# LIA-DiTella/DiffUDF

Hardware: AMD Instinct MI355X
Metric: train points/sec (SIREN fwd+∇x+Eikonal loss+bwd), 256×8 net, 100k pts (higher is better)
Workload: dtype f32

## Files before the change

diffudf_amd/csrc/dudf_sweep_bf16.hip:

```cpp
#include "dudf_sweep16.h"


namespace {

template <int H, int SW, int FL, int SP = 0, int P24 = 0>
__device__ __forceinline__ void sweep_tile_b(const SweepArgs& a, const int g_first, const int nact, char* lds, unsigned& gc,
                                             const bool stamp_on = false) {
    using G = GeoB<H, SP>;
    constexpr int NPC = G::NPC;
    static_assert(SP == 0 || SW <= SWEEP_FWD_J, "fp16x3: plain columns, Hessian quads, jets");
    static_assert(P24 == 0 || ((P24 == 6 || P24 == 7) && SP != 0 && H == 256 && !is_jet(SW)), "24-bit stash arrays (mask 6: R, E, C; 7: S, Q, A, Z as well): the fp16x3 training kernels of 256-wide layers");
    constexpr int BS = base_of(SW);
    constexpr bool HS = is_hess(SW);
    const int tid = threadIdx.x, lane = tid & 63;
    const int wave = __builtin_amdgcn_readfirstlane(tid >> 6);
    const int li = lane & 15, q = lane >> 4;
    const bool isv = !HS || (is_jet(SW) ? li == 0 : (lane & 3) == 0);
    const int nhid = a.L - 1;
    constexpr bool kFwdDir = (BS == SWEEP_FWD || BS == SWEEP_ADJ_FWD);

    f32x4 acc[G::NT], prev[G::NT];
    const int64_t p = (int64_t)(g_first + wave) * 16 + li;
    auto image = [&](int j) -> const char* {
        if constexpr (SP) return kFwdDir ? a.wimg16_f + (size_t)j * G::IMGB : a.wimg16_t + (size_t)(nhid - 1 - j) * G::IMGB;
        return kFwdDir ? a.wimg_f + (size_t)j * G::IMGB : a.wimg_t + (size_t)(nhid - 1 - j) * G::IMGB;
    };
    float unscale = 1.f;
    auto unscale_of = [&](int j) -> float { return a.wsc[kFwdDir ? j : nhid - 1 - j]; };
    constexpr bool kColScale = SP != 0 && (BS != SWEEP_FWD || HS);
    constexpr bool kTrackE = SP != 0 && BS == SWEEP_ADJ_FWD;
    float sb = 1.f, inv_sb = 1.f;
    auto set_scale = [&](float amax_true, float extra, float zb) {
        float bound;
        if constexpr (!HS) { (void)zb; bound = a.w0 * amax_true + extra; }
        else if constexpr (is_jet(SW)) {
            const int l0 = lane & 48;
            const unsigned jw = kJetLane[lane & 15];
            const float w2 = 0.5f * (float)((jw >> 24) & 3), w3 = 0.5f * (float)((jw >> 26) & 3);
            const float F[3] = {a.w0 * __shfl(amax_true, l0 + 1), a.w0 * __shfl(amax_true, l0 + 2), a.w0 * __shfl(amax_true, l0 + 3)};
            auto sel = [&](unsigned k) -> float { k &= 3; return k == 0 ? F[0] : (k == 1 ? F[1] : F[2]); };
            const float S0 = a.w0 * __shfl(amax_true, l0 + (int)(jw & 15)), S1 = a.w0 * __shfl(amax_true, l0 + (int)((jw >> 4) & 15)),
                        S2 = a.w0 * __shfl(amax_true, l0 + (int)((jw >> 8) & 15));
            const float fab = sel(jw >> 18) * sel(jw >> 20);
            const float p2 = S0 * sel(jw >> 12) + S1 * sel(jw >> 14) + S2 * sel(jw >> 16) + w2 * fab;
            const float p3 = w3 * fab * sel(jw >> 22);
            bound = ((jw >> 28) & 1) ? 1.f : a.w0 * amax_true + p3 + p2;
        }
        else if constexpr (BS == SWEEP_FWD) bound = isv ? 1.f : a.w0 * amax_true;
        else if constexpr (BS == SWEEP_REV) {
            const float av = quad_bcast0(amax_true);
            bound = a.w0 * (amax_true + (isv ? 0.f : a.w0 * zb * av));
        } else {
            const float sk = quad_sum(isv ? 0.f : zb * amax_true);
            bound = extra + a.w0 * (amax_true + (isv ? a.w0 * sk : 0.f));
        }
        col_scale(bound * DUDF_FX_HEADROOM, sb, inv_sb);
    };
    auto ebound_of = [&](int layer) -> float {
        if constexpr (kColScale && BS == SWEEP_ADJ_REV && (HS || (FL & 1) != 0)) return a.ebound[(int64_t)layer * a.np + p];
        return 0.f;
    };
    auto zbound_of = [&](int layer) -> float {
        if constexpr (kColScale && HS && BS != SWEEP_FWD) return a.zbound[(int64_t)layer * a.nch + p];
        return 0.f;
    };
    auto store_zbound = [&](int layer, float m) {
        if constexpr (kColScale && HS && !is_jet(SW) && BS == SWEEP_FWD) a.zbound[(int64_t)layer * a.nch + p] = isv ? 0.f : m;
    };
    float eb_next = 0.f, zb_next = 0.f;
    constexpr int kRow = amax_row<SW, FL>();
    constexpr bool kFx = (P24 & 1) != 0;
    TailTrackT<kFx> tmax;
    bool poison = false;
    auto store_fx = [&](int layer) {
        if constexpr (kFx) {
            if constexpr (kColScale) tmax.fs = sb * 0x1p-15f;
            if constexpr (kColScale) a.fxs[(int64_t)layer * a.np + p] = poison ? __uint_as_float(0x7fc00000u) : inv_sb * 0x1p15f;
        }
    };
    unsigned* lds_amax = reinterpret_cast<unsigned*>(lds + amax_lds_off<H, SW, SP>(a));
    auto publish = [&](int layer) {
        if constexpr (kRow >= 0) { lds_max_wave(lds_amax + (layer < kMaxAmaxLayers ? layer : kMaxAmaxLayers - 1), tmax.t); tmax.t = 0.f; }
    };
    auto in_layer = [&](int j) -> int { return kFwdDir ? j : a.L - 1 - j; };
    auto bias_ptr = [&](int layer) -> const float* {
        return a.b1s + (size_t)layer * H;
    };
    auto stash_base = [&](int layer, int T) -> int64_t {
        const int64_t v = (int64_t)layer * a.stash_layer + (int64_t)(16 * T) * a.np;
        const unsigned lo = __builtin_amdgcn_readfirstlane((unsigned)v), hi = __builtin_amdgcn_readfirstlane((unsigned)(v >> 32));
        return (int64_t)(((uint64_t)hi << 32) | lo);
    };
    const unsigned vo = (unsigned)(((int64_t)q * a.np + p) * 16);
    const LaneOff vl(vo, (is_hess(SW) && !is_jet(SW)) ? (unsigned)(((int64_t)q * a.np + (p >> 2)) * 16) : vo,
                     P24 ? (unsigned)(((p >> 4) * 64 + lane) * 12) : 0u,
                     !P24 ? 0u : (is_hess(SW) && !is_jet(SW)) ? (unsigned)(((p >> 6) * 64 + 16 * q + ((p >> 2) & 15)) * 12)
                                                              : (unsigned)(((p >> 4) * 64 + lane) * 12));
    auto load_ops = [&](int layer, int kb, TailOps& o) {
        epilogue_loads<SW, FL, P24>(a, stash_base(layer, 2 * kb), vl, o.o1a, o.o2a, o.o3a);
        epilogue_loads<SW, FL, P24>(a, stash_base(layer, 2 * kb + 1), vl, o.o1b, o.o2b, o.o3b);
        if constexpr (BS == SWEEP_FWD && SP != 0) {
            const float* lb = reinterpret_cast<const float*>(lds + 3 * G::CHUNKB) + layer * H + 32 * kb + 4 * q;
            o.ba = *reinterpret_cast<const f32x4*>(lb);
            o.bb = *reinterpret_cast<const f32x4*>(lb + 16);
        } else if constexpr (BS == SWEEP_FWD) {
            o.ba = *reinterpret_cast<const f32x4*>(bias_ptr(layer) + 32 * kb + 4 * q);
            o.bb = *reinterpret_cast<const f32x4*>(bias_ptr(layer) + 32 * kb + 16 + 4 * q);
        }
    };
    auto run_tail = [&](int layer, int kb, const f32x4 z0, const f32x4 z1, const TailOps& o, f32x4& e0, f32x4& e1) {
        const f32x4 zero = {0, 0, 0, 0};
        if constexpr (BS == SWEEP_FWD && SP != 0 && HS) {
            const f32x4 us = {unscale, unscale, unscale, unscale};
            e0 = epilogue<SW, FL, false, P24, false, TailTrackT<kFx>>(a, __builtin_elementwise_fma(z0, us, isv ? o.ba : zero), zero, zero, zero, stash_base(layer, 2 * kb), vl, isv, tmax);
            e1 = epilogue<SW, FL, false, P24, false, TailTrackT<kFx>>(a, __builtin_elementwise_fma(z1, us, isv ? o.bb : zero), zero, zero, zero, stash_base(layer, 2 * kb + 1), vl, isv, tmax);
        } else if constexpr (BS == SWEEP_FWD && SP != 0) {
            e0 = epilogue<SW, FL, false, P24, false, TailTrackT<kFx>>(a, __builtin_elementwise_fma(z0, f32x4{unscale, unscale, unscale, unscale}, o.ba), zero, zero, zero, stash_base(layer, 2 * kb), vl, isv, tmax);
            e1 = epilogue<SW, FL, false, P24, false, TailTrackT<kFx>>(a, __builtin_elementwise_fma(z1, f32x4{unscale, unscale, unscale, unscale}, o.bb), zero, zero, zero, stash_base(layer, 2 * kb + 1), vl, isv, tmax);
        } else if constexpr (BS == SWEEP_FWD) {
            e0 = epilogue<SW, FL, false, P24, false, TailTrackT<kFx>>(a, z0 + (isv ? o.ba : zero), zero, zero, zero, stash_base(layer, 2 * kb), vl, isv, tmax);
            e1 = epilogue<SW, FL, false, P24, false, TailTrackT<kFx>>(a, z1 + (isv ? o.bb : zero), zero, zero, zero, stash_base(layer, 2 * kb + 1), vl, isv, tmax);
        } else if constexpr (kColScale) {
            e0 = epilogue<SW, FL, kTrackE, P24, false, TailTrackT<kFx>>(a, z0 * unscale, o.o1a, o.o2a, o.o3a, stash_base(layer, 2 * kb), vl, isv, tmax);
            e1 = epilogue<SW, FL, kTrackE, P24, false, TailTrackT<kFx>>(a, z1 * unscale, o.o1b, o.o2b, o.o3b, stash_base(layer, 2 * kb + 1), vl, isv, tmax);
        } else {
            e0 = epilogue<SW, FL, false, P24, false, TailTrackT<kFx>>(a, z0, o.o1a, o.o2a, o.o3a, stash_base(layer, 2 * kb), vl, isv, tmax);
            e1 = epilogue<SW, FL, false, P24, false, TailTrackT<kFx>>(a, z1, o.o1b, o.o2b, o.o3b, stash_base(layer, 2 * kb + 1), vl, isv, tmax);
        }
    };
    auto pin_ops = [&](TailOps& o) {
        if constexpr (BS == SWEEP_FWD) asm volatile("" : "+v"(o.ba), "+v"(o.bb));
        else asm volatile("" : "+v"(o.o1a), "+v"(o.o2a), "+v"(o.o1b), "+v"(o.o2b));
        if constexpr (SW == SWEEP_ADJ_FWD_H || SW == SWEEP_ADJ_REV_H) asm volatile("" : "+v"(o.o3a), "+v"(o.o3b));
    };

    const int total = nhid * G::NKB;
    auto chunk_src = [&](int c) -> const char* {
        const int j = c / G::NKB;
        return image(j) + (size_t)(c - j * G::NKB) * G::CHUNKB;
    };
    __syncthreads();
    const unsigned lds0 = (unsigned)(size_t)(__attribute__((address_space(3))) char*)lds;
    const unsigned voff = (unsigned)lane * 16u;
    auto dma2 = [&](const char* src, unsigned dst) {
        if (wave < NWB / 2) {
            const int w = wave & (NWB / 2 - 1);
            dma_issue<H, SP>(src, dst, voff, w); dma_issue<H, SP>(src, dst, voff, w + NWB / 2);
        }
    };
    dma2(chunk_src(0), lds0 + gc * G::CHUNKB);
    dma2(chunk_src(1), lds0 + ((gc + 1) % 3) * G::CHUNKB);
    if (wave >= nact) {
        dma_wait_b<0>();
        __syncthreads();
        for (int c = 0; c < total; ++c) {
            const bool more = c + 2 < total;
            if (more) dma2(chunk_src(c + 2), lds0 + ((gc + 2) % 3) * G::CHUNKB);
            gc = (gc + 1) % 3;
            if (more) dma_wait_b<2 * G::NDMA>();
            else dma_wait_b<0>();
            __syncthreads();
        }
        return;
    }

    {
        float b = 0.f, yb = 1.f;
        if constexpr (BS == SWEEP_FWD) b = (q < 3) ? a.x4[p * 4 + q] : 0.f;
        if constexpr (BS == SWEEP_ADJ_FWD) b = (q < 3) ? a.gbar[p * 4 + q] : 0.f;
        if constexpr (BS == SWEEP_ADJ_REV) yb = a.ybar[p];
        if constexpr (SW == SWEEP_REV_H) yb = isv ? 1.f : 0.f;
        if constexpr (kFx) {
            if constexpr (BS == SWEEP_REV) poison = nonfinite(a.y[p]);
            if constexpr (BS == SWEEP_ADJ_REV) poison = nonfinite(a.ybar[p]);
            if constexpr (BS == SWEEP_ADJ_FWD) {
                int bad = nonfinite(b) ? 1 : 0;
                bad |= __shfl_xor(bad, 16); bad |= __shfl_xor(bad, 32);
                poison = bad != 0;
            }
        }
#pragma unroll
        for (int T = 0; T < G::NT; ++T) {
            if constexpr (kFwdDir) prev[T] = mfma16(a.w1b[(16 * T + li) * 4 + q], b, f32x4{0, 0, 0, 0});
            else prev[T] = *reinterpret_cast<const f32x4*>(a.theta + a.off_wo + 16 * T + 4 * q) * yb;
        }
    }

    constexpr bool kOneSet = HS;
    TailOps ops_cur, ops_n1;
    u32x4 bp[NPC];
    auto split = [&](const f32x4 e0, const f32x4 e1, u32x4 (&o)[NPC]) {
        if constexpr (kColScale) split8h(e0 * sb, e1 * sb, o[0], o[1]);
        else if constexpr (SP) split8h(e0, e1, o[0], o[1]);
        else split8(e0, e1, o[0], o[1], o[2]);
    };
    auto store_ebound = [&](int layer) {
        if constexpr (kTrackE) {
            float m = fmaxf(tmax.e, __shfl_xor(tmax.e, 16));
            m = fmaxf(m, __shfl_xor(m, 32));
            a.ebound[(int64_t)layer * a.np + p] = m;
            tmax.e = 0.f;
        }
    };
    f32x4 fin0 = {0, 0, 0, 0}, fin1 = {0, 0, 0, 0};
    load_ops(in_layer(0), 0, ops_cur);
    if constexpr (!kOneSet) load_ops(in_layer(0), 1, ops_n1);
    if constexpr (kColScale) {
        const float eb0 = ebound_of(in_layer(0)), zb0 = zbound_of(in_layer(0));
        if (nhid > 0) { eb_next = ebound_of(in_layer(1)); zb_next = zbound_of(in_layer(1)); }
        const float cm = col_absmax(prev);
        store_zbound(in_layer(0), cm);
        set_scale(cm, eb0, zb0);
    }
    store_fx(in_layer(0));
    {
        f32x4 e0, e1;
        run_tail(in_layer(0), 0, prev[0], prev[1], ops_cur, e0, e1);
        split(e0, e1, bp);
        if constexpr (kOneSet) load_ops(in_layer(0), 1, ops_cur);
    }
#pragma unroll
    for (int T = 0; T < G::NT; ++T) acc[T] = f32x4{0, 0, 0, 0};
    dma_wait_b<0>();
    __syncthreads();
    constexpr int kYoung = younger_ops<SW, FL>() - ((SP != 0 && BS == SWEEP_FWD) ? 2 : 0);
    constexpr bool kLateOk = !HS || (SW != SWEEP_ADJ_FWD_H && SW != SWEEP_FWD_J);
    #ifdef DUDF_LATE_FORCE
    const bool late = kLateOk && DUDF_LATE_FORCE;
#else
    const bool late = kLateOk && __builtin_amdgcn_readfirstlane((int)(wave >= NWB / 2)) != 0;
#endif
    constexpr int FA = -1, TA = 0, FB = (BS == SWEEP_FWD ? 15 : 7) * (G::NT - 1) / 15, TB = G::NT - 1;
    for (int j = 0; j < nhid; ++j) {
        const int lin = in_layer(j), lnx = in_layer(j + 1);
#pragma unroll
        for (int kb = 0; kb < G::NKB; ++kb) {
            const int c = j * G::NKB + kb;
            const char* bpl = lds + gc * G::CHUNKB + lane * 16;
            auto frag = [&](int T, int pc) -> u32x4 {
#if DUDF_SWEEP_DBG & 32
                u32x4 z; asm volatile("" : "=v"(z)); return z;
#endif
                return *reinterpret_cast<const u32x4*>(bpl + (T * NPC + pc) * G::FRAG);
            };
            DUDF_STAMP(0);
            if constexpr (!kOneSet) ops_cur = ops_n1;
            pin_ops(ops_cur);
            const bool more = c + 2 < total;
            auto load_after_next = [&](TailOps& o) {
                if (kb + 2 < G::NKB) load_ops(lin, kb + 2, o);
                else load_ops(lnx, kb + 2 - G::NKB, o);
            };
            auto feed = [&]() {
                if (more) dma2(chunk_src(c + 2), lds0 + ((gc + 2) % 3) * G::CHUNKB);
                if constexpr (!kOneSet) load_after_next(ops_n1);
            };
            u32x4 nb[NPC];
            constexpr bool kTailTop = SP != 0 && BS == SWEEP_FWD;
            if (kTailTop && !late && kb + 1 < G::NKB) {
                DUDF_STAMP(2);
                f32x4 e0, e1;
                run_tail(lin, kb + 1, prev[2 * kb + 2], prev[2 * kb + 3], ops_cur, e0, e1);
                split(e0, e1, nb);
                if constexpr (kOneSet) load_after_next(ops_cur);
                DUDF_STAMP(3);
                __builtin_amdgcn_sched_barrier(0);
            }
            if ((FA < 0 && !late) || (FB < 0 && late)) feed();
            DUDF_STAMP(1);
            __builtin_amdgcn_sched_barrier(0);
            constexpr int AD = (SP && BS == SWEEP_FWD) ? 4 : 2;
            u32x4 an[AD][NPC];
#pragma unroll
            for (int T = 0; T < AD; ++T)
#pragma unroll
                for (int pc = 0; pc < NPC; ++pc) an[T][pc] = frag(T, pc);
            constexpr int TP = SP ? 2 : 1;
#pragma unroll
            for (int T = 0; T < G::NT; T += TP) {
                u32x4 af[TP][NPC];
#pragma unroll
                for (int u = 0; u < TP; ++u)
#pragma unroll
                    for (int pc = 0; pc < NPC; ++pc) af[u][pc] = an[(T + u) % AD][pc];
                if (T + AD < G::NT) {
#pragma unroll
                    for (int u = 0; u < TP; ++u)
#pragma unroll
                        for (int pc = 0; pc < NPC; ++pc) an[(T + u) % AD][pc] = frag(T + u + AD, pc);
                    __builtin_amdgcn_sched_barrier(0x76);
                }
                f32x4 cc[TP];
#pragma unroll
                for (int u = 0; u < TP; ++u) cc[u] = acc[T + u];
                if constexpr (SP) {
#pragma unroll
                    for (int u = 0; u < TP; ++u) cc[u] = mfma_h(as_h(af[u][1]), as_h(bp[0]), cc[u]);
#pragma unroll
                    for (int u = 0; u < TP; ++u) cc[u] = mfma_h(as_h(af[u][0]), as_h(bp[1]), cc[u]);
#pragma unroll
                    for (int u = 0; u < TP; ++u) cc[u] = mfma_h(as_h(af[u][0]), as_h(bp[0]), cc[u]);
                } else {
#pragma unroll
                    for (int u = 0; u < TP; ++u) cc[u] = mfma_b(as_bf(af[u][1]), as_bf(bp[1]), cc[u]);
#pragma unroll
                    for (int u = 0; u < TP; ++u) cc[u] = mfma_b(as_bf(af[u][2]), as_bf(bp[0]), cc[u]);
#pragma unroll
                    for (int u = 0; u < TP; ++u) cc[u] = mfma_b(as_bf(af[u][0]), as_bf(bp[2]), cc[u]);
#pragma unroll
                    for (int u = 0; u < TP; ++u) cc[u] = mfma_b(as_bf(af[u][1]), as_bf(bp[0]), cc[u]);
#pragma unroll
                    for (int u = 0; u < TP; ++u) cc[u] = mfma_b(as_bf(af[u][0]), as_bf(bp[1]), cc[u]);
#pragma unroll
                    for (int u = 0; u < TP; ++u) cc[u] = mfma_b(as_bf(af[u][0]), as_bf(bp[0]), cc[u]);
                }
#pragma unroll
                for (int u = 0; u < TP; ++u) acc[T + u] = cc[u];
                const int Tl = T + TP - 1;
                if ((FA >= T && FA <= Tl && !late) || (FB >= T && FB <= Tl && late)) {
                    __builtin_amdgcn_sched_barrier(0);
                    DUDF_STAMP(6);
                    feed();
                    DUDF_STAMP(7);
                    __builtin_amdgcn_sched_barrier(0);
                }
                if (kb + 1 < G::NKB && ((TA >= T && TA <= Tl && !late && !kTailTop) || (TB >= T && TB <= Tl && late))) {
                    if (T != 0) __builtin_amdgcn_sched_barrier(0);
                    DUDF_STAMP(2);
                    f32x4 e0, e1;
                    run_tail(lin, kb + 1, prev[2 * kb + 2], prev[2 * kb + 3], ops_cur, e0, e1);
                    split(e0, e1, nb);
                    if constexpr (kOneSet) load_after_next(ops_cur);
                    DUDF_STAMP(3);
                }
            }
            if (kb + 1 == G::NKB) {
                if constexpr (kColScale) {
                    unscale = unscale_of(j) * inv_sb;
                    const float ebl = eb_next, zbl = zb_next;
                    { const int jn = j + 2 <= nhid ? j + 2 : nhid; eb_next = ebound_of(in_layer(jn)); zb_next = zbound_of(in_layer(jn)); }
                    const float cm = col_absmax(acc) * unscale;
                    store_zbound(lnx, cm);
                    set_scale(cm, ebl, zbl);
                } else if constexpr (SP) unscale = unscale_of(j);
                store_fx(lnx);
                publish(lin);
                store_ebound(lin);
                run_tail(lnx, 0, acc[0], acc[1], ops_cur, fin0, fin1);
                split(fin0, fin1, nb);
                if constexpr (kOneSet) load_after_next(ops_cur);
#pragma unroll
                for (int T = 0; T < G::NT; ++T) { prev[T] = acc[T]; acc[T] = f32x4{0, 0, 0, 0}; }
            }
#pragma unroll
            for (int pc = 0; pc < NPC; ++pc) bp[pc] = nb[pc];
            gc = (gc + 1) % 3;
            DUDF_STAMP(4);
#if !(DUDF_SWEEP_DBG & 8)
            if (more) { if (wave < NWB / 2) dma_wait_b<(kTailTop ? 1 : 2) * kYoung + 2 * G::NDMA>(); }
            else dma_wait_b<0>();
#endif
            DUDF_STAMP(5);
#if !(DUDF_SWEEP_DBG & 16)
            __syncthreads();
#endif
        }
    }

    {
        const int lin = in_layer(nhid);
        float part = 0.f;
        f32x4 accg = {0, 0, 0, 0};
#pragma unroll
        for (int kb = 0; kb < G::NKB; ++kb) {
            f32x4 e0 = fin0, e1 = fin1;
            if (kb > 0) {
                if constexpr (!kOneSet) {
                    ops_cur = ops_n1;
                    if (kb + 1 < G::NKB) load_ops(lin, kb + 1, ops_n1);
                }
                run_tail(lin, kb, prev[2 * kb], prev[2 * kb + 1], ops_cur, e0, e1);
                if constexpr (kOneSet) { if (kb + 1 < G::NKB) load_ops(lin, kb + 1, ops_cur); }
            }
            if constexpr (BS == SWEEP_FWD) {
                const f32x4 w0v = *reinterpret_cast<const f32x4*>(a.theta + a.off_wo + 32 * kb + 4 * q);
                const f32x4 w1v = *reinterpret_cast<const f32x4*>(a.theta + a.off_wo + 32 * kb + 16 + 4 * q);
                part += e0[0] * w0v[0] + e0[1] * w0v[1] + e0[2] * w0v[2] + e0[3] * w0v[3];
                part += e1[0] * w1v[0] + e1[1] * w1v[1] + e1[2] * w1v[2] + e1[3] * w1v[3];
            } else if constexpr (BS == SWEEP_REV) {
                const f32x4 w0v = *reinterpret_cast<const f32x4*>(a.w1t16 + li * H + 32 * kb + 4 * q);
                const f32x4 w1v = *reinterpret_cast<const f32x4*>(a.w1t16 + li * H + 32 * kb + 16 + 4 * q);
#pragma unroll
                for (int t = 0; t < 4; ++t) accg = mfma16(w0v[t], e0[t], accg);
#pragma unroll
                for (int t = 0; t < 4; ++t) accg = mfma16(w1v[t], e1[t], accg);
            }
        }
        publish(lin);
        store_ebound(lin);
        if constexpr (BS == SWEEP_FWD) {
            part += __shfl_xor(part, 16);
            part += __shfl_xor(part, 32);
            if (isv) part += a.theta[a.off_bo];
            if (q == 0) a.y[p] = part;
            if constexpr (kFx) {
                if constexpr (kColScale) {
                    if (q == 0 && nonfinite(part))
                        for (int l = 0; l < a.L; ++l) a.fxs[(int64_t)l * a.np + p] = __uint_as_float(0x7fc00000u);
                } else if (q == 0) {
                    const float sc = nonfinite(part) ? __uint_as_float(0x7fc00000u) : 1.f;
                    for (int l = 0; l < a.L; ++l) a.fxs[(int64_t)l * a.np + p] = sc;
                }
            }
        } else if constexpr (BS == SWEEP_REV) {
            if constexpr (kFx) { if (poison) accg = f32x4{__uint_as_float(0x7fc00000u), __uint_as_float(0x7fc00000u), __uint_as_float(0x7fc00000u), 0.f}; }
            if (q == 0) *reinterpret_cast<f32x4*>(a.g + p * 4) = f32x4{accg[0], accg[1], accg[2], 0.f};
        }
    }
}

template <int H, int SW, int FL, int P24 = 0>
__device__ __forceinline__ void sweep_tile_oct(const SweepArgs& a, const int g, char* lds, unsigned& gc, const unsigned oct_off) {
    using G = GeoB<H, 1>;
    static_assert(H == 256 && SW <= SWEEP_ADJ_REV, "fp16x3, plain columns, one k-block per wave");
    constexpr int NPC = 2;
    constexpr int BS = base_of(SW);
    const int tid = threadIdx.x, lane = tid & 63;
    const int wave = __builtin_amdgcn_readfirstlane(tid >> 6);
    const int li = lane & 15, q = lane >> 4;
    const int nhid = a.L - 1;
    constexpr bool kFwdDir = (BS == SWEEP_FWD || BS == SWEEP_ADJ_FWD);
    constexpr bool kColScale = BS != SWEEP_FWD;
    constexpr bool kTrackE = BS == SWEEP_ADJ_FWD;
    constexpr int kRow = amax_row<SW, FL>();
    const int64_t p = (int64_t)g * 16 + li;
    const int T0 = 2 * wave;
    auto image = [&](int j) -> const char* {
        return kFwdDir ? a.wimg16_f + (size_t)j * G::IMGB : a.wimg16_t + (size_t)(nhid - 1 - j) * G::IMGB;
    };
    auto unscale_of = [&](int j) -> float { return a.wsc[kFwdDir ? j : nhid - 1 - j]; };
    auto in_layer = [&](int j) -> int { return kFwdDir ? j : a.L - 1 - j; };
    auto stash_base = [&](int layer, int T) -> int64_t {
        const int64_t v = (int64_t)layer * a.stash_layer + (int64_t)(16 * T) * a.np;
        const unsigned lo = __builtin_amdgcn_readfirstlane((unsigned)v), hi = __builtin_amdgcn_readfirstlane((unsigned)(v >> 32));
        return (int64_t)(((uint64_t)hi << 32) | lo);
    };
    const LaneOff vo((unsigned)(((int64_t)q * a.np + p) * 16), (unsigned)(((int64_t)q * a.np + p) * 16),
                     P24 ? (unsigned)(((p >> 4) * 64 + lane) * 12) : 0u);
    char* ox = lds + oct_off;
    u32x4* Bx = reinterpret_cast<u32x4*>(ox);
    float* cmx = reinterpret_cast<float*>(ox + 8 * NPC * 1024);
    float* emx = cmx + 128;
    f32x4* red = reinterpret_cast<f32x4*>(ox + 8 * NPC * 1024 + 1024);
    unsigned* lds_amax = reinterpret_cast<unsigned*>(lds + 3 * G::CHUNKB);

    (void)gc;
    __syncthreads();

    f32x4 prev[2], acc[2];
    bool poison = false;
    {
        float b = 0.f, yb = 1.f;
        if constexpr (BS == SWEEP_FWD) b = (q < 3) ? a.x4[p * 4 + q] : 0.f;
        if constexpr (BS == SWEEP_ADJ_FWD) b = (q < 3) ? a.gbar[p * 4 + q] : 0.f;
        if constexpr (BS == SWEEP_ADJ_REV) yb = a.ybar[p];
        if constexpr ((P24 & 1) != 0) {
            if constexpr (BS == SWEEP_REV) poison = nonfinite(a.y[p]);
            if constexpr (BS == SWEEP_ADJ_REV) poison = nonfinite(yb);
            if constexpr (BS == SWEEP_ADJ_FWD) {
                int bad = nonfinite(b) ? 1 : 0;
                bad |= __shfl_xor(bad, 16); bad |= __shfl_xor(bad, 32);
                poison = bad != 0;
            }
        }
#pragma unroll
        for (int u = 0; u < 2; ++u) {
            const int T = T0 + u;
            if constexpr (kFwdDir) prev[u] = mfma16(a.w1b[(16 * T + li) * 4 + q], b, f32x4{0, 0, 0, 0});
            else prev[u] = *reinterpret_cast<const f32x4*>(a.theta + a.off_wo + 16 * T + 4 * q) * yb;
        }
    }
    f32x4 o1[2], o2[2], o3[2], bs[2] = {{0, 0, 0, 0}, {0, 0, 0, 0}};
    auto load_ops = [&](int layer) {
#pragma unroll
        for (int u = 0; u < 2; ++u) {
            epilogue_loads<SW, FL, P24>(a, stash_base(layer, T0 + u), vo, o1[u], o2[u], o3[u]);
            if constexpr (BS == SWEEP_FWD)
                bs[u] = *reinterpret_cast<const f32x4*>(reinterpret_cast<const float*>(lds + 3 * G::CHUNKB) + layer * H + 16 * (T0 + u) + 4 * q);
        }
    };
    auto ebound_of = [&](int layer) -> float {
        if constexpr (BS == SWEEP_ADJ_REV && (FL & 1) != 0) return a.ebound[(int64_t)layer * a.np + p];
        return 0.f;
    };
    load_ops(in_layer(0));
    float eb = ebound_of(in_layer(0));
    float unscale = 1.f, sb = 1.f, inv_sb = 1.f;
    constexpr bool kFx = (P24 & 1) != 0;
    TailTrackT<kFx> tk;
    f32x4 e[2];
    for (int j = 0; j <= nhid; ++j) {
        const int lin = in_layer(j);
        if constexpr (kColScale) {
            const float m = col_absmax(prev);
            if (q == 0) cmx[wave * 16 + li] = m;
            __syncthreads();
            float mm = 0.f;
#pragma unroll
            for (int w = 0; w < NWB; ++w) mm = fmaxf(mm, cmx[w * 16 + li]);
            col_scale((a.w0 * (mm * unscale) + eb) * DUDF_FX_HEADROOM, sb, inv_sb);
        }
        if constexpr (kFx) {
            if constexpr (kColScale) tk.fs = sb * 0x1p-15f;
            if (wave == 0 && q == 0) a.fxs[(int64_t)lin * a.np + p] = poison ? __uint_as_float(0x7fc00000u) : (kColScale ? inv_sb * 0x1p15f : 1.f);
        }
#pragma unroll
        for (int u = 0; u < 2; ++u) {
            f32x4 z = prev[u];
            if constexpr (BS == SWEEP_FWD) z = __builtin_elementwise_fma(z, f32x4{unscale, unscale, unscale, unscale}, bs[u]);
            else z *= unscale;
            e[u] = epilogue<SW, FL, kTrackE, P24, false, TailTrackT<kFx>>(a, z, o1[u], o2[u], o3[u], stash_base(lin, T0 + u), vo, true, tk);
        }
        if constexpr (kRow >= 0) { if (lin < kMaxAmaxLayers) lds_max_wave(lds_amax + lin, tk.t); tk.t = 0.f; }
        if constexpr (kTrackE) {
            float m = fmaxf(tk.e, __shfl_xor(tk.e, 16));
            m = fmaxf(m, __shfl_xor(m, 32));
            if (q == 0) emx[wave * 16 + li] = m;
            tk.e = 0.f;
        }
        if (j == nhid) break;
        u32x4 fr[G::NKB][2][NPC];
        {
            const char* img = image(j) + (size_t)lane * 16;
#pragma unroll
            for (int kb = 0; kb < G::NKB; ++kb)
#pragma unroll
                for (int u = 0; u < 2; ++u)
#pragma unroll
                    for (int pc = 0; pc < NPC; ++pc)
                        fr[kb][u][pc] = *reinterpret_cast<const u32x4*>(img + (size_t)kb * G::CHUNKB + ((T0 + u) * NPC + pc) * G::FRAG);
        }
        u32x4 bh, bl;
        if constexpr (kColScale) split8h(e[0] * sb, e[1] * sb, bh, bl);
        else split8h(e[0], e[1], bh, bl);
        Bx[(wave * NPC + 0) * 64 + lane] = bh;
        Bx[(wave * NPC + 1) * 64 + lane] = bl;
        load_ops(in_layer(j + 1));
        eb = ebound_of(in_layer(j + 1));
        __syncthreads();
        if constexpr (kTrackE) {
            if (wave == 0 && q == 0 && a.ebound) {
                float m = 0.f;
#pragma unroll
                for (int w = 0; w < NWB; ++w) m = fmaxf(m, emx[w * 16 + li]);
                a.ebound[(int64_t)lin * a.np + p] = m;
            }
        }
        acc[0] = f32x4{0, 0, 0, 0}; acc[1] = acc[0];
#pragma unroll
        for (int kb = 0; kb < G::NKB; ++kb) {
            const u32x4 b0 = Bx[(kb * NPC + 0) * 64 + lane], b1 = Bx[(kb * NPC + 1) * 64 + lane];
#pragma unroll
            for (int u = 0; u < 2; ++u) {
                f32x4 cc = acc[u];
                cc = mfma_h(as_h(fr[kb][u][1]), as_h(b0), cc);
                cc = mfma_h(as_h(fr[kb][u][0]), as_h(b1), cc);
                cc = mfma_h(as_h(fr[kb][u][0]), as_h(b0), cc);
                acc[u] = cc;
            }
        }
        __syncthreads();
        prev[0] = acc[0]; prev[1] = acc[1];
        unscale = kColScale ? unscale_of(j) * inv_sb : unscale_of(j);
    }
    if constexpr (BS == SWEEP_FWD) {
        float part = 0.f;
#pragma unroll
        for (int u = 0; u < 2; ++u) {
            const f32x4 wv = *reinterpret_cast<const f32x4*>(a.theta + a.off_wo + 16 * (T0 + u) + 4 * q);
            part += e[u][0] * wv[0] + e[u][1] * wv[1] + e[u][2] * wv[2] + e[u][3] * wv[3];
        }
        part += __shfl_xor(part, 16);
        part += __shfl_xor(part, 32);
        if (q == 0) cmx[wave * 16 + li] = part;
        __syncthreads();
        if (wave == 0 && q == 0) {
            float y = a.theta[a.off_bo];
#pragma unroll
            for (int w = 0; w < NWB; ++w) y += cmx[w * 16 + li];
            a.y[p] = y;
            if constexpr (kFx) {
                if (nonfinite(y))
                    for (int l = 0; l < a.L; ++l) a.fxs[(int64_t)l * a.np + p] = __uint_as_float(0x7fc00000u);
            }
        }
    } else if constexpr (BS == SWEEP_REV) {
        f32x4 accg = {0, 0, 0, 0};
#pragma unroll
        for (int u = 0; u < 2; ++u) {
            const f32x4 wv = *reinterpret_cast<const f32x4*>(a.w1t16 + li * H + 16 * (T0 + u) + 4 * q);
#pragma unroll
            for (int t = 0; t < 4; ++t) accg = mfma16(wv[t], e[u][t], accg);
        }
        red[wave * 64 + lane] = accg;
        __syncthreads();
        if (wave == 0 && q == 0) {
            f32x4 sum = {0, 0, 0, 0};
#pragma unroll
            for (int w = 0; w < NWB; ++w) sum += red[w * 64 + lane];
            if constexpr (kFx) { if (poison) sum = f32x4{__uint_as_float(0x7fc00000u), __uint_as_float(0x7fc00000u), __uint_as_float(0x7fc00000u), 0.f}; }
            *reinterpret_cast<f32x4*>(a.g + p * 4) = f32x4{sum[0], sum[1], sum[2], 0.f};
        }
    } else if constexpr (kTrackE) {
        __syncthreads();
        if (wave == 0 && q == 0 && a.ebound) {
            float m = 0.f;
#pragma unroll
            for (int w = 0; w < NWB; ++w) m = fmaxf(m, emx[w * 16 + li]);
            a.ebound[(int64_t)in_layer(nhid) * a.np + p] = m;
        }
    }
}

template <int H, int SW, int FL, int SP = 0, int P24 = 0>
__device__ __forceinline__ void sweep_body_b(const SweepArgs& a, const int bid, const int nblk) {
    extern __shared__ __attribute__((aligned(16))) char lds_b[];
    unsigned gc = 0;
    const bool clk_on = a.clk != nullptr && bid == 0;
    const unsigned long long clk_t0 = clk_on ? __builtin_amdgcn_s_memtime() : 0ull, clk_r0 = clk_on ? __builtin_amdgcn_s_memrealtime() : 0ull;
    constexpr int kRow = amax_row<SW, FL>();
    unsigned* lds_amax = reinterpret_cast<unsigned*>(lds_b + amax_lds_off<H, SW, SP>(a));
    if constexpr (kRow >= 0) { if (threadIdx.x < kMaxAmaxLayers) lds_amax[threadIdx.x] = 0u; }
    if constexpr (SP != 0 && base_of(SW) == SWEEP_FWD) {
        float* lb = reinterpret_cast<float*>(lds_b + 3 * GeoB<H, SP>::CHUNKB);
        for (int i = threadIdx.x; i < a.L * H; i += 64 * NWB) lb[i] = a.b1s[i];
    }
    const int ng = a.ntiles * (TILE / 16), gbase = a.tile0 * (TILE / 16);
    const int g0 = (int)((int64_t)bid * ng / nblk), g1 = (int)((int64_t)(bid + 1) * ng / nblk);
    constexpr bool kOct = SP != 0 && H == 256 && SW <= SWEEP_ADJ_REV;
    for (int g = g0; g < g1; g += NWB) {
        if constexpr (kOct) {
            if (g1 - g == 1) {
                const unsigned oct_off = 3 * GeoB<H, SP>::CHUNKB + (base_of(SW) == SWEEP_FWD ? (unsigned)(a.L * H * sizeof(float)) : (unsigned)(kMaxAmaxLayers * sizeof(unsigned)));
                sweep_tile_oct<H, SW, FL, P24>(a, gbase + g, lds_b, gc, oct_off);
                continue;
            }
        }
        sweep_tile_b<H, SW, FL, SP, P24>(a, gbase + g, (g1 - g < NWB) ? g1 - g : NWB, lds_b, gc, (DUDF_SWEEP_DBG & 128) && bid == 100 && g == g0);
    }
    if constexpr (kRow >= 0) {
        __syncthreads();
        if ((int)threadIdx.x < a.L && (int)threadIdx.x < kMaxAmaxLayers && a.amax) {
            const unsigned v = lds_amax[threadIdx.x];
            if (v) atomicMax(a.amax + kRow * a.L + threadIdx.x, v);
        }
    }
    if (clk_on && threadIdx.x == 0) {
        a.clk[0] = __builtin_amdgcn_s_memtime() - clk_t0;
        a.clk[1] = __builtin_amdgcn_s_memrealtime() - clk_r0;
    }
}
template <int H, int SW, int FL>
__global__ __launch_bounds__(64 * NWB) void sweep_bf16_kernel(SweepArgs a) { sweep_body_b<H, SW, FL>(a, blockIdx.x, gridDim.x); }
template <int H, int SW, int FL>
__global__ __launch_bounds__(64 * NWB) DUDF_NO_PK void sweep_bf16_np_kernel(SweepArgs a) { sweep_body_b<H, SW, FL>(a, blockIdx.x, gridDim.x); }
template <int H, int SW, int FL>
__global__ __launch_bounds__(64 * NWB) void sweep_f16_kernel(SweepArgs a) { sweep_body_b<H, SW, FL, 1>(a, blockIdx.x, gridDim.x); }
template <int H, int SW, int FL>
__global__ __launch_bounds__(64 * NWB) DUDF_NO_PK void sweep_f16_np_kernel(SweepArgs a) { sweep_body_b<H, SW, FL, 1>(a, blockIdx.x, gridDim.x); }
template <int H, int SW, int FL>
__global__ __launch_bounds__(64 * NWB) void sweep_f16r_kernel(SweepArgs a) { sweep_body_b<H, SW, FL, 1, 6>(a, blockIdx.x, gridDim.x); }
template <int H, int SW, int FL>
__global__ __launch_bounds__(64 * NWB) DUDF_NO_PK void sweep_f16r_np_kernel(SweepArgs a) { sweep_body_b<H, SW, FL, 1, 6>(a, blockIdx.x, gridDim.x); }
template <int H, int SW, int FL>
__global__ __launch_bounds__(64 * NWB) void sweep_f16p_kernel(SweepArgs a) { sweep_body_b<H, SW, FL, 1, 7>(a, blockIdx.x, gridDim.x); }
template <int H, int SW, int FL>
__global__ __launch_bounds__(64 * NWB) DUDF_NO_PK void sweep_f16p_np_kernel(SweepArgs a) { sweep_body_b<H, SW, FL, 1, 7>(a, blockIdx.x, gridDim.x); }
template <int H, int SWQ, int FLQ, int SWP, int FLP, int SPQ, int P24 = 0>
__global__ __launch_bounds__(64 * NWB) DUDF_NO_PK void sweep_pair_kernel(SweepArgs aq, SweepArgs ap, int nbq) {
    if ((int)blockIdx.x < nbq) sweep_body_b<H, SWQ, FLQ, SPQ, P24>(aq, blockIdx.x, nbq);
    else sweep_body_b<H, SWP, FLP, 1, P24>(ap, (int)blockIdx.x - nbq, (int)gridDim.x - nbq);
}

template <int H, int FAM, int SW, int FL>
constexpr auto sweep_kernel_of() {
    constexpr bool np = sweep_no_pk<SW>();
    if constexpr (FAM == DUDF_FAM_BF16) { if constexpr (np) return &sweep_bf16_np_kernel<H, SW, FL>; else return &sweep_bf16_kernel<H, SW, FL>; }
    else if constexpr (FAM == DUDF_FAM_F16) { if constexpr (np) return &sweep_f16_np_kernel<H, SW, FL>; else return &sweep_f16_kernel<H, SW, FL>; }
    else if constexpr (FAM == DUDF_FAM_F16R) { if constexpr (np) return &sweep_f16r_np_kernel<H, SW, FL>; else return &sweep_f16r_kernel<H, SW, FL>; }
    else { if constexpr (np) return &sweep_f16p_np_kernel<H, SW, FL>; else return &sweep_f16p_kernel<H, SW, FL>; }
}
static_assert(dudf_chunk_bytes(256, 3) == GeoB<256>::CHUNKB && dudf_chunk_bytes(128, 2) == GeoB<128, 1>::CHUNKB, "dudf_variants.h: LDS sizes");
template <int H>
int launch_b(const SweepChoice& c, const SweepArgs& a, hipStream_t st) {
    if (a.ntiles <= 0) return 0;
    const int ntb = (a.ntiles * TILE + TILEB - 1) / TILEB;
    const dim3 grid(ntb < 256 ? ntb : 256), block(GeoB<H>::NTHR);
    return dudf_with_variant(kSweepVariants, c.sw, c.fl, [&](auto i) {
        constexpr DudfVariant v = kSweepVariants[decltype(i)::value];
        if (c.family == DUDF_FAM_BF16) return dudf_launch_kernel<sweep_kernel_of<H, DUDF_FAM_BF16, v.sw, v.fl>()>(grid, block, c.lds, c.lds_max, st, a);
        if (c.family == DUDF_FAM_F16) return dudf_launch_kernel<sweep_kernel_of<H, DUDF_FAM_F16, v.sw, v.fl>()>(grid, block, c.lds, c.lds_max, st, a);
        if constexpr (H == 256 && v.p24 != 0) {
            if (c.family == DUDF_FAM_F16R) return dudf_launch_kernel<sweep_kernel_of<H, DUDF_FAM_F16R, v.sw, v.fl>()>(grid, block, c.lds, c.lds_max, st, a);
            if (c.family == DUDF_FAM_F16P) return dudf_launch_kernel<sweep_kernel_of<H, DUDF_FAM_F16P, v.sw, v.fl>()>(grid, block, c.lds, c.lds_max, st, a);
        }
        return (int)DUDF_E_UNSUPPORTED;
    });
}

double pair_est(int ng, int nb, double c) {
    const int m = (ng + nb - 1) / nb, full = m / NWB, rem = m % NWB;
    const double part = rem == 0 ? 0.0 : (rem <= NWB / 2 ? 0.55 : 0.55 + 0.45 * (rem - NWB / 2) / (NWB / 2));
    return c * (full + part);
}
}

int dudf_launch_sweep_pair(const SweepChoice& c, const SweepArgs& aq, const SweepArgs& ap, hipStream_t st) {
    const int ngq = aq.ntiles * (TILE / 16), ngp = ap.ntiles * (TILE / 16);
    const int tq = (ngq + NWB - 1) / NWB, tp = (ngp + NWB - 1) / NWB;
    int nbq, nbp;
    if (tq + tp <= 256) { nbq = tq; nbp = tp; }
    else {
        double best = 1e30; nbq = 128;
        for (int q = 1; q < 256; ++q) {
            const double eq = pair_est(ngq, q, 1.5), ep = pair_est(ngp, 256 - q, 1.0);
            const double t = (eq > ep ? eq : ep) + 1e-3 * (eq > ep ? eq - ep : ep - eq);
            if (t < best) { best = t; nbq = q; }
        }
        nbp = 256 - nbq;
    }
    const dim3 grid(nbq + nbp), block(GeoB<256>::NTHR);
    return dudf_with_variant(kPairVariants, c.sw, c.fl, [&](auto i) {
        constexpr DudfVariant v = kPairVariants[decltype(i)::value];
        auto go = [&](auto spq, auto p24) {
            return dudf_launch_kernel<&sweep_pair_kernel<256, v.sw + 4, dudf_pair_flq(v.sw), v.sw, v.fl, decltype(spq)::value, decltype(p24)::value>>(
                grid, block, c.lds, c.lds_max, st, aq, ap, nbq);
        };
        using std::integral_constant;
        if (c.p24 == 7) return go(integral_constant<int, 1>{}, integral_constant<int, 7>{});
        if (c.p24 == 6) return go(integral_constant<int, 1>{}, integral_constant<int, 6>{});
        if (c.spq) return go(integral_constant<int, 1>{}, integral_constant<int, 0>{});
        return go(integral_constant<int, 0>{}, integral_constant<int, 0>{});
    });
}

int dudf_launch_sweep_bf16(const SweepChoice& c, const SweepArgs& a, hipStream_t st) {
    switch (c.H) {
        case 256: return launch_b<256>(c, a, st);
        case 128: return launch_b<128>(c, a, st);
        case 512: return dudf_launch_sweep_wide(c, a, st);
        default: return DUDF_E_UNSUPPORTED;
    }
}

#if DUDF_FX_CHECK
int dudf_fx_read_wide(unsigned* out2, int reset);
extern "C" int dudf_dbg_fx_violations(unsigned* out2, int reset) {
    out2[0] = out2[1] = 0u;
    const int e = dudf_fx_read(out2, reset);
    return e ? e : dudf_fx_read_wide(out2, reset);
}
#endif
```

Baseline: 39.82 million.

## Software-pipeline weight fragment loads and LDS double-buffer in oct sweep tile

Restructures the single-group (oct) sweep path so the next layer's weight fragments are loaded while the current layer's MFMAs run, with the first layer's fragments and epilogue operands prefetched before the loop. B-operand reads from LDS are also prefetched one k-block ahead and the MFMAs for both tiles are interleaved. In the forward sweep the LDS staging buffer alternates between two regions, which drops the trailing barrier. The cost is higher register pressure from holding fragments across iterations and reuse of LDS offset 0 as a second buffer, which must not collide with other data. A debug flag that skips the regular tile path is also added.

```diff
diff --git a/diffudf_amd/csrc/dudf_sweep_bf16.hip b/diffudf_amd/csrc/dudf_sweep_bf16.hip
--- a/diffudf_amd/csrc/dudf_sweep_bf16.hip
+++ b/diffudf_amd/csrc/dudf_sweep_bf16.hip
@@ -425,7 +425,9 @@
     static_assert(H == 256 && SW <= SWEEP_ADJ_REV, "fp16x3, plain columns, one k-block per wave");
     constexpr int NPC = 2;
     constexpr int BS = base_of(SW);
-    const int tid = threadIdx.x, lane = tid & 63;
+    int tid = threadIdx.x;
+    asm volatile("" : "+v"(tid));
+    const int lane = tid & 63;
     const int wave = __builtin_amdgcn_readfirstlane(tid >> 6);
     const int li = lane & 15, q = lane >> 4;
     const int nhid = a.L - 1;
@@ -449,6 +451,7 @@
                      P24 ? (unsigned)(((p >> 4) * 64 + lane) * 12) : 0u);
     char* ox = lds + oct_off;
     u32x4* Bx = reinterpret_cast<u32x4*>(ox);
+    u32x4* Bx1 = reinterpret_cast<u32x4*>(lds);
     float* cmx = reinterpret_cast<float*>(ox + 8 * NPC * 1024);
     float* emx = cmx + 128;
     f32x4* red = reinterpret_cast<f32x4*>(ox + 8 * NPC * 1024 + 1024);
@@ -457,15 +460,55 @@
     (void)gc;
     __syncthreads();
 
+    struct OctOps { f32x4 o1[2], o2[2], o3[2], bs[2]; float eb; };
+    auto ebound_of = [&](int layer) -> float {
+        if constexpr (BS == SWEEP_ADJ_REV && (FL & 1) != 0) return a.ebound[(int64_t)layer * a.np + p];
+        return 0.f;
+    };
+    auto load_ops = [&](int layer, OctOps& o) {
+#pragma unroll
+        for (int u = 0; u < 2; ++u) {
+            epilogue_loads<SW, FL, P24>(a, stash_base(layer, T0 + u), vo, o.o1[u], o.o2[u], o.o3[u]);
+            if constexpr (BS == SWEEP_FWD)
+                o.bs[u] = *reinterpret_cast<const f32x4*>(reinterpret_cast<const float*>(lds + 3 * G::CHUNKB) + layer * H + 16 * (T0 + u) + 4 * q);
+        }
+        o.eb = ebound_of(layer);
+    };
+    u32x4 fr[G::NKB][2][NPC];
+    auto load_frags = [&](int j, int kb) {
+        const char* img = image(j) + (size_t)lane * 16 + (size_t)kb * G::CHUNKB;
+#pragma unroll
+        for (int u = 0; u < 2; ++u)
+#pragma unroll
+            for (int pc = 0; pc < NPC; ++pc)
+                fr[kb][u][pc] = *reinterpret_cast<const u32x4*>(img + ((T0 + u) * NPC + pc) * G::FRAG);
+    };
+
     f32x4 prev[2], acc[2];
     bool poison = false;
+    OctOps ops = {};
     {
         float b = 0.f, yb = 1.f;
         if constexpr (BS == SWEEP_FWD) b = (q < 3) ? a.x4[p * 4 + q] : 0.f;
         if constexpr (BS == SWEEP_ADJ_FWD) b = (q < 3) ? a.gbar[p * 4 + q] : 0.f;
         if constexpr (BS == SWEEP_ADJ_REV) yb = a.ybar[p];
+        float poison_y = 0.f;
+        if constexpr ((P24 & 1) != 0 && BS == SWEEP_REV) poison_y = a.y[p];
+        float w1v[2] = {0.f, 0.f};
+        f32x4 wov[2] = {{0, 0, 0, 0}, {0, 0, 0, 0}};
+#pragma unroll
+        for (int u = 0; u < 2; ++u) {
+            const int T = T0 + u;
+            if constexpr (kFwdDir) w1v[u] = a.w1b[(16 * T + li) * 4 + q];
+            else wov[u] = *reinterpret_cast<const f32x4*>(a.theta + a.off_wo + 16 * T + 4 * q);
+        }
+        load_ops(in_layer(0), ops);
+        __builtin_amdgcn_sched_barrier(0);
+#pragma unroll
+        for (int kb = 0; kb < G::NKB; ++kb) load_frags(0, kb);
+        __builtin_amdgcn_sched_barrier(0);
         if constexpr ((P24 & 1) != 0) {
-            if constexpr (BS == SWEEP_REV) poison = nonfinite(a.y[p]);
+            if constexpr (BS == SWEEP_REV) poison = nonfinite(poison_y);
             if constexpr (BS == SWEEP_ADJ_REV) poison = nonfinite(yb);
             if constexpr (BS == SWEEP_ADJ_FWD) {
                 int bad = nonfinite(b) ? 1 : 0;
@@ -475,31 +518,17 @@
         }
 #pragma unroll
         for (int u = 0; u < 2; ++u) {
-            const int T = T0 + u;
-            if constexpr (kFwdDir) prev[u] = mfma16(a.w1b[(16 * T + li) * 4 + q], b, f32x4{0, 0, 0, 0});
-            else prev[u] = *reinterpret_cast<const f32x4*>(a.theta + a.off_wo + 16 * T + 4 * q) * yb;
-        }
-    }
-    f32x4 o1[2], o2[2], o3[2], bs[2] = {{0, 0, 0, 0}, {0, 0, 0, 0}};
-    auto load_ops = [&](int layer) {
-#pragma unroll
-        for (int u = 0; u < 2; ++u) {
-            epilogue_loads<SW, FL, P24>(a, stash_base(layer, T0 + u), vo, o1[u], o2[u], o3[u]);
-            if constexpr (BS == SWEEP_FWD)
-                bs[u] = *reinterpret_cast<const f32x4*>(reinterpret_cast<const float*>(lds + 3 * G::CHUNKB) + layer * H + 16 * (T0 + u) + 4 * q);
-        }
-    };
-    auto ebound_of = [&](int layer) -> float {
-        if constexpr (BS == SWEEP_ADJ_REV && (FL & 1) != 0) return a.ebound[(int64_t)layer * a.np + p];
-        return 0.f;
-    };
-    load_ops(in_layer(0));
-    float eb = ebound_of(in_layer(0));
+            if constexpr (kFwdDir) prev[u] = mfma16(w1v[u], b, f32x4{0, 0, 0, 0});
+            else prev[u] = wov[u] * yb;
+        }
+    }
     float unscale = 1.f, sb = 1.f, inv_sb = 1.f;
+    float wsc_j = unscale_of(0);
     constexpr bool kFx = (P24 & 1) != 0;
     TailTrackT<kFx> tk;
     f32x4 e[2];
     for (int j = 0; j <= nhid; ++j) {
+        OctOps& o = ops;
         const int lin = in_layer(j);
         if constexpr (kColScale) {
             const float m = col_absmax(prev);
@@ -508,7 +537,7 @@
             float mm = 0.f;
 #pragma unroll
             for (int w = 0; w < NWB; ++w) mm = fmaxf(mm, cmx[w * 16 + li]);
-            col_scale((a.w0 * (mm * unscale) + eb) * DUDF_FX_HEADROOM, sb, inv_sb);
+            col_scale((a.w0 * (mm * unscale) + o.eb) * DUDF_FX_HEADROOM, sb, inv_sb);
         }
         if constexpr (kFx) {
             if constexpr (kColScale) tk.fs = sb * 0x1p-15f;
@@ -517,9 +546,9 @@
 #pragma unroll
         for (int u = 0; u < 2; ++u) {
             f32x4 z = prev[u];
-            if constexpr (BS == SWEEP_FWD) z = __builtin_elementwise_fma(z, f32x4{unscale, unscale, unscale, unscale}, bs[u]);
+            if constexpr (BS == SWEEP_FWD) z = __builtin_elementwise_fma(z, f32x4{unscale, unscale, unscale, unscale}, o.bs[u]);
             else z *= unscale;
-            e[u] = epilogue<SW, FL, kTrackE, P24, false, TailTrackT<kFx>>(a, z, o1[u], o2[u], o3[u], stash_base(lin, T0 + u), vo, true, tk);
+            e[u] = epilogue<SW, FL, kTrackE, P24, false, TailTrackT<kFx>>(a, z, o.o1[u], o.o2[u], o.o3[u], stash_base(lin, T0 + u), vo, true, tk);
         }
         if constexpr (kRow >= 0) { if (lin < kMaxAmaxLayers) lds_max_wave(lds_amax + lin, tk.t); tk.t = 0.f; }
         if constexpr (kTrackE) {
@@ -529,24 +558,18 @@
             tk.e = 0.f;
         }
         if (j == nhid) break;
-        u32x4 fr[G::NKB][2][NPC];
-        {
-            const char* img = image(j) + (size_t)lane * 16;
-#pragma unroll
-            for (int kb = 0; kb < G::NKB; ++kb)
-#pragma unroll
-                for (int u = 0; u < 2; ++u)
-#pragma unroll
-                    for (int pc = 0; pc < NPC; ++pc)
-                        fr[kb][u][pc] = *reinterpret_cast<const u32x4*>(img + (size_t)kb * G::CHUNKB + ((T0 + u) * NPC + pc) * G::FRAG);
-        }
         u32x4 bh, bl;
         if constexpr (kColScale) split8h(e[0] * sb, e[1] * sb, bh, bl);
         else split8h(e[0], e[1], bh, bl);
-        Bx[(wave * NPC + 0) * 64 + lane] = bh;
-        Bx[(wave * NPC + 1) * 64 + lane] = bl;
-        load_ops(in_layer(j + 1));
-        eb = ebound_of(in_layer(j + 1));
+        const u32x4* Bj = (BS == SWEEP_FWD && (j & 1)) ? Bx1 : Bx;
+        {
+            u32x4* Bw = (BS == SWEEP_FWD && (j & 1)) ? Bx1 : Bx;
+            Bw[(wave * NPC + 0) * 64 + lane] = bh;
+            Bw[(wave * NPC + 1) * 64 + lane] = bl;
+        }
+        load_ops(in_layer(j + 1), o);
+        const float wsc_cur = wsc_j;
+        wsc_j = unscale_of(j + 1 < nhid ? j + 1 : j);
         __syncthreads();
         if constexpr (kTrackE) {
             if (wave == 0 && q == 0 && a.ebound) {
@@ -557,21 +580,29 @@
             }
         }
         acc[0] = f32x4{0, 0, 0, 0}; acc[1] = acc[0];
-#pragma unroll
-        for (int kb = 0; kb < G::NKB; ++kb) {
-            const u32x4 b0 = Bx[(kb * NPC + 0) * 64 + lane], b1 = Bx[(kb * NPC + 1) * 64 + lane];
-#pragma unroll
-            for (int u = 0; u < 2; ++u) {
-                f32x4 cc = acc[u];
-                cc = mfma_h(as_h(fr[kb][u][1]), as_h(b0), cc);
-                cc = mfma_h(as_h(fr[kb][u][0]), as_h(b1), cc);
-                cc = mfma_h(as_h(fr[kb][u][0]), as_h(b0), cc);
-                acc[u] = cc;
-            }
-        }
-        __syncthreads();
+        auto multiply = [&](auto refill) {
+            u32x4 b0 = Bj[(0 * NPC + 0) * 64 + lane], b1 = Bj[(0 * NPC + 1) * 64 + lane];
+#pragma unroll
+            for (int kb = 0; kb < G::NKB; ++kb) {
+                u32x4 n0 = b0, n1 = b1;
+                if (kb + 1 < G::NKB) { n0 = Bj[((kb + 1) * NPC + 0) * 64 + lane]; n1 = Bj[((kb + 1) * NPC + 1) * 64 + lane]; }
+                f32x4 c0 = acc[0], c1 = acc[1];
+                c0 = mfma_h(as_h(fr[kb][0][1]), as_h(b0), c0);
+                c1 = mfma_h(as_h(fr[kb][1][1]), as_h(b0), c1);
+                c0 = mfma_h(as_h(fr[kb][0][0]), as_h(b1), c0);
+                c1 = mfma_h(as_h(fr[kb][1][0]), as_h(b1), c1);
+                c0 = mfma_h(as_h(fr[kb][0][0]), as_h(b0), c0);
+                c1 = mfma_h(as_h(fr[kb][1][0]), as_h(b0), c1);
+                acc[0] = c0; acc[1] = c1;
+                if constexpr (decltype(refill)::value) load_frags(j + 1, kb);
+                __builtin_amdgcn_sched_barrier(0);
+                b0 = n0; b1 = n1;
+            }
+        };
+        if (j + 1 < nhid) multiply(std::true_type{});
+        else multiply(std::false_type{});
         prev[0] = acc[0]; prev[1] = acc[1];
-        unscale = kColScale ? unscale_of(j) * inv_sb : unscale_of(j);
+        unscale = kColScale ? wsc_cur * inv_sb : wsc_cur;
     }
     if constexpr (BS == SWEEP_FWD) {
         float part = 0.f;
@@ -646,6 +677,7 @@
                 continue;
             }
         }
+        if constexpr ((DUDF_SWEEP_DBG & 256) != 0) continue;
         sweep_tile_b<H, SW, FL, SP, P24>(a, gbase + g, (g1 - g < NWB) ? g1 - g : NWB, lds_b, gc, (DUDF_SWEEP_DBG & 128) && bid == 100 && g == g0);
     }
     if constexpr (kRow >= 0) {
```

Measured after the change: 40.01 million, median of 6. About the same (+0.5%).
